# anonymous-author-918/deq-mpc-corl

Hardware: AMD Instinct MI355X
Metric: QP solves/sec at (B,T=20,nx=13,nu=4) (higher is better)
Workload: dtype f32

## Files before the change

### deq-mpc-corl_amd/csrc/alqp_quad.hip

```cpp
#include <hip/hip_runtime.h>

#include "alqp_quad.hpp"
#include "alqp_dims.hpp"
#include "alqp_launch.hpp"

#if defined(ALQP_QUAD_F32) == defined(ALQP_QUAD_F64)
#error "compile alqp_quad.hip with exactly one of -DALQP_QUAD_F32, -DALQP_QUAD_F64"
#endif

namespace alqp {

#ifndef ALQP_FUSE_LS
#define ALQP_FUSE_LS 1
#endif
#ifdef ALQP_PHASE_TIMING
__device__ unsigned long long g_phase_cycles[10];
#define QSTAMP(b) qd.stamp(b)
#else
#define QSTAMP(b)
#endif
template <typename real, int NX, int NU, bool TRACE, class Dyn = NoDyn>
__global__ __launch_bounds__(64) __attribute__((amdgpu_waves_per_eu(1, 1))) void k_solve_lin_quad(SolveArgs<real> a, TraceArgs<real> tr, real *ws) {
    using C = QCfg<real, NX, NU>;
    constexpr bool NL = Dyn::ID != 0;
#ifndef ALQP_FUSE_LS_F64
#define ALQP_FUSE_LS_F64 1
#endif
    constexpr bool FUSE_LS = ALQP_FUSE_LS && (sizeof(real) == 4 || ALQP_FUSE_LS_F64) && !NL;
    constexpr int N = C::N;
    if (a.skip && *a.skip != 0.0) return;
    const int lane = threadIdx.x, qi = lane >> 2;
    const int b_raw = blockIdx.x * 16 + qi;
    const bool active = b_raw < a.B;
    {
        int stag = a.stagger;
        const int mode = (a.flags >> 20) & 0xf;
        if ((a.flags >> 24) & 0xff) stag = (a.flags >> 24) & 0xff;
        if (stag > 0) {
            const unsigned hw = __builtin_amdgcn_s_getreg(4 | (0 << 6) | (31 << 11));
            int simd = (hw >> 4) & 3;
            if (mode == 1) simd = simd * 16 + ((hw >> 8) & 0xf);
            if (mode == 2) simd &= 1;
            if (mode == 3) simd = blockIdx.x & 1;
            if (mode == 4) simd = (simd & 1) ^ (blockIdx.x & 1);
            if (mode == 5) simd = (hw >> 8) & 3;
            for (int i = 0; i < simd * stag; ++i) __builtin_amdgcn_s_sleep(16);
        }
    }
#ifdef ALQP_ALIAS_ALL
    const int b = (active ? b_raw : a.B - 1) % ALQP_ALIAS_ALL;
#else
    const int b = active ? b_raw : a.B - 1;
#endif
    const int T = a.T, M = C::M(T);

    Quad<real, NX, NU> qd;
    __shared__ real w_lds[QCfg<real, NX, NU>::WLDS_WORDS];
    qd.wl = w_lds + threadIdx.x;
    qd.q = lane & 3;
    qd.T = T;
    qd.active = active;
    qd.gQd = a.Qd + (size_t)b * T * N;
    qd.gq = a.q + (size_t)b * T * N;
    qd.gF = a.F + (size_t)b * (T - 1) * NX * N;
    qd.gc = a.c + (size_t)b * (T - 1) * NX;
    qd.gx0 = a.x0 + (size_t)b * NX;
    qd.gulo = a.ulo + (size_t)b * a.sb_u;
    qd.guhi = a.uhi + (size_t)b * a.sb_u;
    qd.st_u = a.st_u;
    qd.gz = a.z + (size_t)b * T * N;
    qd.glam = a.lam + (size_t)b * M;
    qd.rec = ws + C::rec_base(b, T);
    qd.gFw = const_cast<real *>(qd.gF);
    qd.dyn_h = a.dyn_h;
    qd.rho = a.rho[b];
    qd.info = 0;
    real phi_prev = a.phi[b];
#ifdef ALQP_PHASE_TIMING
    for (int i = 0; i < 10; ++i) qd.tacc[i] = 0;
#endif
    QSTAMP(-1);
    if (!(a.flags & ALQP_WS_PRIMED)) {
        if constexpr (NL) qd.stage_in(false, false);
        else qd.stage_in(a.max_newton == 0 || a.al_iter == 0 || (a.flags & ALQP_EXIT_IN_KERNEL) ||
                         (!C::PHI0_FWD && (a.flags & ALQP_INIT_MERIT)));
    }
    const bool ref_exit = (a.flags & ALQP_EXIT_IN_KERNEL) != 0;
    int gphase = 0;

    int step_id = 0;
    bool pend = false;
// ... 84 lines not shown
        if (ref_exit && a.newton_counts && blockIdx.x == 0 && lane == 0) a.newton_counts[it] = grid_barrier_timed_out(a.exit_scratch) ? -1 : n_done;
        bad = 0;
        qd.template iter_end<Dyn>(alpha_pend, pend, (a.flags & ALQP_DUAL_UPDATE) != 0, (real)a.rho_scale, it + 1 == a.al_iter,
                    phi_next, rn2, bad);
        pend = false;
    }
    if (a.al_iter <= 0) {
        rn2 = qd.rplus2(bad);
        qd.stage_out();
    }
#ifdef ALQP_PHASE_TIMING
    QSTAMP(9);
    if (lane == 0)
        for (int i = 0; i < 10; ++i) atomicAdd(&g_phase_cycles[i], qd.tacc[i]);
#endif
    if (active && qd.q == 0) {
        a.rho[b] = qd.rho;
        a.phi[b] = phi_prev;
        if (a.rnorm2) a.rnorm2[b] = rn2;
        if (a.info && qd.info && a.info[b] == 0) a.info[b] = qd.info;
        if (a.status) a.status[b] = bad ? 0 : 1;
    }
}

template <typename real, int NX, int NU>
__global__ __launch_bounds__(64) __attribute__((amdgpu_waves_per_eu(1, 1))) void k_backward_quad(BwdArgs<real> a, real *ws) {
    using C = QCfg<real, NX, NU>;
    constexpr int N = C::N;
    const int lane = threadIdx.x, qi = lane >> 2;
    const int b_raw = blockIdx.x * 16 + qi;
    const bool active = b_raw < a.B;
    const int b = active ? b_raw : a.B - 1;
    const int T = a.T;
    Quad<real, NX, NU> qd;
    __shared__ real w_lds[QCfg<real, NX, NU>::WLDS_WORDS];
    qd.wl = w_lds + threadIdx.x;
    qd.q = lane & 3;
    qd.T = T;
    qd.active = active;
    qd.gF = a.F + (size_t)b * (T - 1) * NX * N;
    qd.gQd = nullptr; qd.gq = nullptr; qd.gc = nullptr; qd.gx0 = nullptr; qd.gulo = nullptr; qd.guhi = nullptr;
    qd.st_u = 0;
    qd.gz = nullptr; qd.glam = nullptr;
    qd.rec = ws + C::rec_base(b, T);
    qd.rho = a.rho[b];
    qd.info = 0;
    qd.solve_forward(a.gbar + (size_t)b * T * N);
    real unused[20];
    qd.template backward<false>(unused);
    if (active) {
        const real *zf = a.z_final + (size_t)b * T * N;
        real *qg = a.q_grad + (size_t)b * T * N;
        real *Qg = a.Qd_grad + (size_t)b * T * N;
        for (int t = 0; t < T; ++t)
            for (int j = qd.q; j < N; j += 4) {
                const real w = qd.recp(t)[C::wn(C::oY, j)];
                qg[t * N + j] = w;
                Qg[t * N + j] = w * zf[t * N + j];
            }
    }
}

template <typename real, int NX, int NU>
__global__ __launch_bounds__(64) __attribute__((amdgpu_waves_per_eu(1, 1))) void k_newton_step_quad(StepArgs<real> a, real *ws) {
    using C = QCfg<real, NX, NU>;
    constexpr int N = C::N, SW = C::SW;
    const int lane = threadIdx.x, qi = lane >> 2;
    const int b_raw = blockIdx.x * 16 + qi;
    const bool active = b_raw < a.B;
    const int b = active ? b_raw : a.B - 1;
    const int T = a.T, M = C::M(T) + T * a.nobs;
    Quad<real, NX, NU> qd;
    __shared__ real w_lds[QCfg<real, NX, NU>::WLDS_WORDS];
    qd.wl = w_lds + threadIdx.x;
    qd.q = lane & 3;
    qd.T = T;
    qd.active = active;
    qd.gQd = a.Qd + (size_t)b * T * N;
    qd.gq = a.q + (size_t)b * T * N;
    qd.gF = a.F + (size_t)b * (T - 1) * NX * N;
    qd.gc = nullptr;
    qd.gx0 = a.x0 + (size_t)b * NX;
    qd.gulo = a.ulo + (size_t)b * a.sb_u;
    qd.guhi = a.uhi + (size_t)b * a.sb_u;
    qd.st_u = a.st_u;
    qd.gz = const_cast<real *>(a.z) + (size_t)b * T * N;
    qd.glam = const_cast<real *>(a.lam) + (size_t)b * M;
    qd.rec = ws + C::rec_base(b, T);
    qd.gFw = const_cast<real *>(qd.gF);
    qd.dyn_h = 0;
    qd.rho = a.rho[b];
    qd.info = 0;
    qd.nobs = a.nobs;
    qd.gobs = a.nobs > 0 ? a.obs + (size_t)b * T * a.nobs * 3 : nullptr;
    qd.obs_r2 = a.obs_r2;
    qd.no_init = a.no_init != 0;
    const real *gxn = a.xnext + (size_t)b * (T - 1) * NX;
    real *tg = (a.g_out && active) ? a.g_out + (size_t)b * T * N : nullptr;
    qd.template forward<true>(tg, real(0), false, nullptr, gxn);
    real unused[20];
    qd.template backward<false>(unused, a.d_out + (size_t)b * T * N);
    if (active) {
        if (qd.q == 0 && a.info && qd.info && a.info[b] == 0) a.info[b] = qd.info;
    }
}


// ... 69 lines not shown
```

### deq-mpc-corl_amd/csrc/alqp_quad.hpp

```cpp
#pragma once
#include <hip/hip_runtime.h>

#include <type_traits>

#include "alqp_team.hpp"
#include "alqp_dyn.hpp"

namespace alqp {

template <int Q>
__device__ inline float qb(float v) {
    return __builtin_bit_cast(float, __builtin_amdgcn_mov_dpp(__builtin_bit_cast(int, v), Q * 0x55, 0xF, 0xF, true));
}
template <int Q>
__device__ inline double qb(double v) {
    long long b = __builtin_bit_cast(long long, v);
    int lo = __builtin_amdgcn_mov_dpp((int)(b & 0xffffffffll), Q * 0x55, 0xF, 0xF, true);
    int hi = __builtin_amdgcn_mov_dpp((int)(b >> 32), Q * 0x55, 0xF, 0xF, true);
    return __builtin_bit_cast(double, ((long long)hi << 32) | (unsigned int)lo);
}
template <typename real>
__device__ inline real qbv(real v, int src) {
    switch (src & 3) {
        case 0: return qb<0>(v);
        case 1: return qb<1>(v);
        case 2: return qb<2>(v);
        default: return qb<3>(v);
    }
}
template <int CTRL>
__device__ inline float qperm(float v) {
    return __builtin_bit_cast(float, __builtin_amdgcn_mov_dpp(__builtin_bit_cast(int, v), CTRL, 0xF, 0xF, true));
}
template <int CTRL>
__device__ inline double qperm(double v) {
    long long b = __builtin_bit_cast(long long, v);
    int lo = __builtin_amdgcn_mov_dpp((int)(b & 0xffffffffll), CTRL, 0xF, 0xF, true);
    int hi = __builtin_amdgcn_mov_dpp((int)(b >> 32), CTRL, 0xF, 0xF, true);
    return __builtin_bit_cast(double, ((long long)hi << 32) | (unsigned int)lo);
}
template <typename real>
__device__ inline real qsum(real v) {
    v += qperm<0xB1>(v);
    v += qperm<0x4E>(v);
    return v;
}
__device__ inline int qor(int v) {
    v |= __builtin_amdgcn_mov_dpp(v, 0xB1, 0xF, 0xF, true);
    v |= __builtin_amdgcn_mov_dpp(v, 0x4E, 0xF, 0xF, true);
    return v;
}
template <typename real>
__device__ inline real sel4(real a0, real a1, real a2, real a3, int q) {
    real lo = (q & 1) ? a1 : a0, hi = (q & 1) ? a3 : a2;
    return (q & 2) ? hi : lo;
}

struct __attribute__((packed, aligned(4))) f4u { float x, y, z, w; };
struct __attribute__((packed, aligned(8))) d4u { double x, y, z, w; };
__device__ inline void gld4(const float *p, float &a, float &b, float &c, float &d) {
    f4u t = *reinterpret_cast<const f4u *>(p);
// ... 1 lines not shown
}
__device__ inline void gld4(const double *p, double &a, double &b, double &c, double &d) {
    d4u t = *reinterpret_cast<const d4u *>(p);
    a = t.x; b = t.y; c = t.z; d = t.w;
}
__device__ inline void gst4(float *p, float a, float b, float c, float d) {
    f4u t; t.x = a; t.y = b; t.z = c; t.w = d;
    *reinterpret_cast<f4u *>(p) = t;
}
__device__ inline void gst4(double *p, double a, double b, double c, double d) {
    d4u t; t.x = a; t.y = b; t.z = c; t.w = d;
    *reinterpret_cast<d4u *>(p) = t;
}
template <int LEN, typename real>
__device__ inline void gload(const real *p, real (&dst)[LEN]) {
#pragma unroll
    for (int c = 0; c + 4 <= LEN; c += 4) gld4(p + c, dst[c], dst[c + 1], dst[c + 2], dst[c + 3]);
#pragma unroll
    for (int c = (LEN / 4) * 4; c < LEN; ++c) dst[c] = p[c];
}

#ifndef ALQP_W_LDS
#define ALQP_W_LDS 1
#endif
#ifndef ALQP_EXP_NOQ
#define ALQP_EXP_NOQ 0
#endif
#ifndef ALQP_EXP_NORS
#define ALQP_EXP_NORS 0
#endif
#ifndef ALQP_EXP_NOL
#define ALQP_EXP_NOL 0
#endif
template <typename real, int SW, int N, bool IN_LDS>
struct WPanel {
    real a[SW][N];
    __device__ __forceinline__ real (&operator[](int s))[N] { return a[s]; }
    __device__ __forceinline__ const real (&operator[](int s) const)[N] { return a[s]; }
};
template <typename real, int N>
struct WRowLds {
    real *p;
    __device__ __forceinline__ real &operator[](int k) const { return p[k * 64]; }
};
template <typename real, int SW, int N>
struct WPanel<real, SW, N, true> {
    real *base;
    __device__ __forceinline__ WRowLds<real, N> operator[](int s) const { return WRowLds<real, N>{base + s * N * 64}; }
};
template <int LEN, typename real>
__device__ __forceinline__ void gload(const real *p, WRowLds<real, LEN> row) {
    real tmp[LEN];
    gload<LEN>(p, tmp);
#pragma unroll
    for (int k = 0; k < LEN; ++k) row[k] = tmp[k];
}

struct NoDyn {
    static constexpr int ID = 0;
};

struct Fld {
    int h, t;
};
template <int H, int T>
struct FldT {
// ... 15 lines not shown
    static constexpr int NX = NX_, NU = NU_, N = NX_ + NU_;
    static constexpr int SH = (N + 3) / 4;
    static constexpr int SW = (NX + 3) / 4;
    static constexpr int SY = SH;
    static constexpr int HT = 2 * SH * (SH + 1);
    __host__ __device__ static constexpr int hidx(int s, int j) { return 2 * s * (s + 1) + j; }
    static constexpr int ST = 2 * SW * (SW + 1);
    static constexpr int BLK = 64 / (int)sizeof(real);
#ifndef ALQP_REC_IL_F32
#define ALQP_REC_IL_F32 2
#endif
    static constexpr int IL = sizeof(real) == 4 ? ALQP_REC_IL_F32 : 1;
    static_assert(IL == 1 || BLK == 16, "groups of 16 words are 64-byte blocks");
    __host__ __device__ static constexpr int w(int x) { return (x / 16) * (16 * IL) + x % 16; }
    static constexpr int NLAST = N - 4 * (SH - 1);
    __host__ __device__ static constexpr int lanes_of(int s) { return s == SH - 1 ? NLAST : 4; }
    __host__ __device__ static constexpr int lstride(int s) { return lanes_of(s) == 3 ? 16 : 4 * lanes_of(s); }
    __host__ __device__ static constexpr int lbase(int s) {
        int o = 0;
        for (int i = 0; i < s; ++i) o += (i + 1) * lstride(i);
        return o;
    }
    static constexpr int LW = lbase(SH);
    static constexpr bool PHI0_FWD = sizeof(real) == 4;
#ifndef ALQP_S_AFTER_F32
#define ALQP_S_AFTER_F32 0
#endif
    static constexpr bool S_AFTER = sizeof(real) == 8 || ALQP_S_AFTER_F32;
#ifndef ALQP_W_LDS_F32
#define ALQP_W_LDS_F32 0
#endif
    static constexpr bool W_LDS = ALQP_W_LDS && (sizeof(real) == 8 || ALQP_W_LDS_F32);
    static constexpr int WLDS_WORDS = W_LDS ? SW * N * 64 : 1;
    __host__ __device__ static constexpr int p4(int x) { return (x + 3) & ~3; }
    static constexpr int NF = 9;
    __host__ __device__ static constexpr int fslots(int i) { return (i <= 1 || i == 6 || i == 7) ? SY : (i == 5 ? 4 : SW); }
    static constexpr int oL = 2 * 16 * (SY / 4);
    __host__ __device__ static constexpr int tail_at(int i) {
        int g = (oL + LW + 15) & ~15, o = 0;
        for (int k = 0; k < NF; ++k) {
            const int r = fslots(k) % 4;
            if (r > 0 && o + r > 4) { g += 16; o = 0; }
            if (k == i) return g + o;
            o += r;
        }
        return o > 0 ? g + 16 : g;
    }
    __host__ __device__ static constexpr int head_at(int i) {
        if (i < 2) return i * 16 * (SY / 4);
        int o = tail_at(NF);
        for (int k = 2; k < i; ++k) o += 16 * (fslots(k) / 4);
        return o;
    }
    static constexpr FldT<head_at(0), tail_at(0)> oY{};
    static constexpr FldT<head_at(1), tail_at(1)> oZ{};
    static constexpr FldT<head_at(2), tail_at(2)> oR{};
    static constexpr FldT<head_at(3), tail_at(3)> oS{};
    static constexpr FldT<head_at(4), tail_at(4)> oLE{};
    static_assert(NU <= 4, "the u-slot layout holds one control per lane");
    static constexpr FldT<head_at(5), tail_at(5)> oUS{};
    static constexpr FldT<head_at(6), tail_at(6)> oQ{};
    static constexpr FldT<head_at(7), tail_at(7)> oq{};
    static constexpr FldT<head_at(8), tail_at(8)> oC{};
    static constexpr int RECW = (head_at(NF) + 31) & ~31;
    static_assert(IL == 1 || RECW % 16 == 0, "whole groups per record");
    template <int S>
    __host__ __device__ static constexpr int lp(int m, int q) {
        return m < 4 * (S / 4) ? 16 * (m / 4) + 4 * q + m % 4 : 16 * (S / 4) + q * (S % 4) + m - 4 * (S / 4);
    }
    template <int S>
    __host__ __device__ static constexpr int fw(Fld f, int p) {
        return p < 16 * (S / 4) ? w(f.h + p) : w(f.t + 4 * ((p - 16 * (S / 4)) / (S % 4)) + (p - 16 * (S / 4)) % (S % 4));
    }
    __host__ __device__ static constexpr int pn(int k) { return lp<SY>(k >> 2, k & 3); }
    __host__ __device__ static constexpr int px(int r) { return lp<SW>(r >> 2, r & 3); }
    __host__ __device__ static constexpr int wn(Fld f, int k) { return fw<SY>(f, pn(k)); }
    __host__ __device__ static constexpr int M(int T) { return T * NX + 2 * T * NU; }
    static constexpr int RSTR = RECW * IL;
    __host__ __device__ static constexpr size_t rec_base(int b, int T) { return (size_t)(b / IL) * T * RSTR + (size_t)(b % IL) * 16; }
    __host__ __device__ static constexpr size_t ws_words(int B, int T) { return (size_t)((B + IL - 1) / IL) * T * RSTR; }
    __host__ static bool ws_covers(int B, int T) {
        return rec_base(B - 1, T) + (size_t)(T - 1) * RSTR + w(RECW - 1) + 1 <= ws_words(B, T);
    }
};

template <typename real, int NX, int NU>
struct Quad {
    using C = QCfg<real, NX, NU>;
    static constexpr int N = C::N, SH = C::SH, SW = C::SW, SY = C::SY, HT = C::HT, ST = C::ST, RECW = C::RECW;

    int q, T;
    bool active;
    const real *gQd, *gq, *gF, *gc, *gx0, *gulo, *guhi;
    long st_u;
    real *gz, *glam, *rec;
    real rho;
    int info;
    real *wl;
    using WT = WPanel<real, SW, N, C::W_LDS>;
    __device__ __forceinline__ WT wpanel() const {
        if constexpr (C::W_LDS) return WT{wl};
        else return WT{};
    }
    real *gFw;
    real dyn_h;
    const real *gobs;
    int nobs;
    real obs_r2;
    bool no_init;

    __device__ __forceinline__ real uhi(int t, int j) const { return guhi[t * st_u + j]; }
    __device__ __forceinline__ real ulo(int t, int j) const { return gulo[t * st_u + j]; }
    __device__ __forceinline__ real *recp(int t) const { return rec + (size_t)t * C::RSTR; }
#ifdef ALQP_PHASE_TIMING
    unsigned long long tacc[10], tlast;
    __device__ __forceinline__ void stamp(int bucket) {
        unsigned long long now;
        __builtin_amdgcn_sched_barrier(0);
        asm volatile("s_waitcnt vmcnt(0)\n\ts_memtime %0\n\ts_waitcnt lgkmcnt(0)" : "=s"(now)::"memory");
        __builtin_amdgcn_sched_barrier(0);
        if (bucket >= 0) tacc[bucket] += now - tlast;
        tlast = now;
// ... 88 lines not shown
        for (int m = 0; m < SL; ++m) {
            const int k = 4 * m + q;
            const real x = src[(4 * m + 3 < LEN || k < LEN) ? k : LEN - 1];
            v[m] = (4 * m + 3 < LEN || k < LEN) ? x : real(0);
        }
    }
    template <int LEN, int SL>
    __device__ __forceinline__ void st_own_ext(real *dst, const real (&v)[SL]) const {
#pragma unroll
        for (int m = 0; m < SL; ++m)
            if (4 * m + 3 < LEN || 4 * m + q < LEN) dst[4 * m + q] = v[m];
    }

    __device__ __forceinline__ int own_ju() const { return (q - NX) & 3; }
    __device__ __forceinline__ void ld_own_us(const real *rp, real &lu, real &ll, real &bu, real &bl) const {
        gld4(rp + C::w(C::oUS.h) + 4 * q, lu, ll, bu, bl);
    }
    __device__ __forceinline__ void st_own_us(real *rp, real lu, real ll, real bu, real bl) const {
        gst4(rp + C::w(C::oUS.h) + 4 * q, lu, ll, bu, bl);
    }
    __device__ __forceinline__ void ld_rep_us(const real *rp, real (&lu)[NU], real (&ll)[NU], real (&bu)[NU], real (&bl)[NU]) const {
        real w[16];
        ld_field<4>(rp + C::oUS, w);
#pragma unroll
        for (int ju = 0; ju < NU; ++ju) {
            const int ql = (NX + ju) & 3;
            lu[ju] = w[4 * ql];
            ll[ju] = w[4 * ql + 1];
            bu[ju] = w[4 * ql + 2];
            bl[ju] = w[4 * ql + 3];
        }
    }

    __device__ __forceinline__ void load_F_rows(int t, WT &W) const {
        const real *Fg = gF + (size_t)t * NX * N;
#pragma unroll
        for (int s = 0; s < SW; ++s) {
            const int r = 4 * s + q;
            const int rc = (4 * s + 3 < NX) ? r : (r < NX ? r : NX - 1);
            gload<N>(Fg + rc * N, W[s]);
            if (4 * s + 3 >= NX) {
                const real m = r < NX ? real(1) : real(0);
#pragma unroll
                for (int k = 0; k < N; ++k) W[s][k] *= m;
            }
        }
    }
    template <int LEN>
    __device__ __forceinline__ void copy_slice(const real *src, real *dst) const {
#pragma unroll
        for (int c = 0; 16 * c < LEN; ++c) {
            const int w0 = 16 * c + 4 * q;
            if (16 * c + 15 < LEN || w0 + 3 < LEN) {
                real a, b, cc, d;
                gld4(src + w0, a, b, cc, d);
                gst4(dst + w0, a, b, cc, d);
            } else {
#pragma unroll
                for (int w = 0; w < 4; ++w)
                    if (w0 + w < LEN) dst[w0 + w] = src[w0 + w];
            }
        }
    }
    __device__ __forceinline__ void stage_in(bool with_residual, bool have_c = true) {
#pragma unroll 2
        for (int t = 0; t < T; ++t) {
            const bool dyn = t < T - 1;
            real *rp = recp(t);
            if (active) {
                real vn[SY], vx[SW];
                ld_own_ext<N>(gz + t * N, vn);
                st_own_n(rp + C::oZ, vn);
                ld_own_ext<N>(gQd + t * N, vn);
                st_own_n(rp + C::oQ, vn);
                ld_own_ext<N>(gq + t * N, vn);
                st_own_n(rp + C::oq, vn);
                ld_own_ext<NX>(glam + t * NX, vx);
                st_own_x(rp + C::oLE, vx);
                {
                    const int ju = own_ju(), jc = ju < NU ? ju : 0;
                    const real *lb = glam + T * NX + t * 2 * NU;
                    const real a0 = lb[jc], a1 = lb[NU + jc], a2 = guhi[t * st_u + jc], a3 = gulo[t * st_u + jc];
                    const bool has = ju < NU;
                    st_own_us(rp, has ? a0 : real(0), has ? a1 : real(0), has ? a2 : real(0), has ? a3 : real(0));
                }
                if (dyn && have_c) ld_own_ext<NX>(gc + t * NX, vx);
                else {
#pragma unroll
                    for (int s = 0; s < SW; ++s) vx[s] = 0;
                }
                if (have_c) st_own_x(rp + C::oC, vx);
            }
            if (with_residual) {
                WT W = wpanel();
                real zt[N];
                load_F_rows(dyn ? t : (T > 1 ? T - 2 : 0), W);
                gload<N>(gz + t * N, zt);
                real rr[SW];
#pragma unroll
                for (int s = 0; s < SW; ++s) {
                    const int r = 4 * s + q;
                    rr[s] = 0;
                    if (4 * s + 3 < NX || r < NX) {
                        real xn = dyn ? gc[t * NX + r] : real(0);
#pragma unroll
                        for (int k = 0; k < N; ++k) xn = fma_(W[s][k], zt[k], xn);
                        rr[s] = dyn ? gz[(t + 1) * N + r] - xn : gz[r] - gx0[r];
                    }
                }
                if (active) st_own_x(rp + C::oR, rr);
            }
        }
    }
    __device__ __forceinline__ void stage_out() {
        if (!active) return;
#pragma unroll 2
        for (int t = 0; t < T; ++t) {
            const real *rp = recp(t);
            real vn[SY], vx[SW];
            ld_own_n(rp + C::oZ, vn);
            st_own_ext<N>(gz + t * N, vn);
            ld_own_x(rp + C::oLE, vx);
            st_own_ext<NX>(glam + t * NX, vx);
            {
                real lu, ll, bu, bl;
                ld_own_us(rp, lu, ll, bu, bl);
                const int ju = own_ju();
                if (ju < NU) {
                    glam[T * NX + t * 2 * NU + ju] = lu;
                    glam[T * NX + t * 2 * NU + NU + ju] = ll;
// ... 145 lines not shown
#pragma unroll
        for (int s = 0; s < SW; ++s) Sy[s] = 0;
        {
            real z0[SW], xi[SW], li[SW], r0[SW];
            if constexpr (EXT) {
                ld_own_ext<NX>(gz, z0);
                ld_own_ext<NX>(glam + (T - 1) * NX, li);
            } else {
                ld_ownx_of_n(recp(0) + C::oZ, z0);
                ld_own_x(recp(T - 1) + C::oLE, li);
            }
            ld_own_ext<NX>(gx0, xi);
            if (pending) {
                real d0[SW];
                ld_ownx_of_n(recp(0) + C::oY, d0);
#pragma unroll
                for (int s = 0; s < SW; ++s) z0[s] = fma_(alpha, d0[s], z0[s]);
            }
#pragma unroll
            for (int s = 0; s < SW; ++s) {
                bool valid = 4 * s + 3 < NX || 4 * s + q < NX;
                if constexpr (EXT) valid = valid && !no_init;
                const real r = valid ? z0[s] - xi[s] : real(0);
                vpo[s] = valid ? fma_(rho, r, li[s]) : real(0);
                if constexpr (C::PHI0_FWD) mdist += valid ? fma_(fma_(real(0.5) * rho, r, li[s]), r, real(0)) : real(0);
                Syo[s] = 0;
                r0[s] = r;
            }
            if (!EXT && active) st_own_x(recp(T - 1) + C::oR, r0);
        }
        for (int t = 0; t < T; ++t) {
            const bool dyn = t < T - 1;
            WT W = wpanel();
            real Y[N];
            real dio[SY];
            real v[SW];
            real zs[SY];
            real hob[3] = {0, 0, 0};
            real *rp = recp(t);
            {
                real zt[N];
                real Qo[SY], qo[SY];
                real cs[SW], zn[SW], lm[SW];
                real lu, ll, bu, bl;
                const int td = dyn ? t : (T > 1 ? T - 2 : 0);
                const real *rn = recp(td + 1);
                if constexpr (EXT) {
                    ld_own_ext<N>(gz + t * N, zs);
                    ld_own_ext<N>(gQd + t * N, Qo);
                    ld_own_ext<N>(gq + t * N, qo);
                    load_F_rows(td, W);
                    ld_own_ext<NX>(gxn + td * NX, cs);
                    ld_own_ext<NX>(gz + (td + 1) * N, zn);
                    ld_own_ext<NX>(glam + td * NX, lm);
                    const int ju = own_ju(), jc = ju < NU ? ju : 0;
                    const real *lb = glam + T * NX + t * (2 * NU + nobs);
                    const bool has = ju < NU;
                    lu = has ? lb[jc] : real(0);
                    ll = has ? lb[NU + jc] : real(0);
                    bu = has ? guhi[t * st_u + jc] : real(0);
                    bl = has ? gulo[t * st_u + jc] : real(0);
                } else {
                    ld_own_n(rp + C::oZ, zs);
                    if constexpr (ALQP_EXP_NOQ) { for (int m = 0; m < SY; ++m) Qo[m] = real(1); }
                    else ld_own_n(rp + C::oQ, Qo);
                    ld_own_n(rp + C::oq, qo);
                    load_F_rows(td, W);
                    ld_own_x(rp + C::oC, cs);
                    ld_ownx_of_n(rn + C::oZ, zn);
                    ld_own_x(rp + C::oLE, lm);
                    ld_own_us(rp, lu, ll, bu, bl);
                }
                if (pending) {
                    real dt[SY], dn[SW];
                    ld_own_n(rp + C::oY, dt);
                    ld_ownx_of_n(rn + C::oY, dn);
#pragma unroll
                    for (int m = 0; m < SY; ++m) zs[m] = fma_(alpha, dt[m], zs[m]);
#pragma unroll
                    for (int s = 0; s < SW; ++s) zn[s] = fma_(alpha, dn[s], zn[s]);
                }
                ALQP_STAMP(0);
#pragma unroll
                for (int k = 0; k < N; ++k) zt[k] = qbv(zs[k >> 2], k);
                real rro[SW];
                if (!dyn) {
#pragma unroll
                    for (int s = 0; s < SW; ++s)
#pragma unroll
                        for (int k = 0; k < N; ++k) W[s][k] = 0;
                }
#pragma unroll
                for (int s = 0; s < SW; ++s) {
                    const int r = 4 * s + q;
                    real xn = cs[s];
                    if constexpr (!EXT) {
#pragma unroll
                        for (int k = 0; k < N; ++k) xn = fma_(W[s][k], zt[k], xn);
                    }
                    const real rr = zn[s] - xn;
                    const bool ok = dyn && r < NX;
                    v[s] = ok ? fma_(rho, rr, lm[s]) : real(0);
                    rro[s] = ok ? rr : real(0);
                    if constexpr (C::PHI0_FWD) mdist += ok ? fma_(fma_(real(0.5) * rho, rr, lm[s]), rr, real(0)) : real(0);
                }
                if (!ALQP_EXP_NORS && !EXT && dyn && active) st_own_x(rp + C::oR, rro);
                constexpr int MU0 = NX / 4;
                real zu = 0;
#pragma unroll
                for (int m = MU0; m < SY; ++m) zu = (4 * m + q >= NX && 4 * m + q < N) ? zs[m] : zu;
                const real vu = zu - bu, vl = bl - zu;
                const real au = vu >= 0 ? real(1) : real(0), al = vl >= 0 ? real(1) : real(0);
                const real cu = fmax_(vu, real(0)), cl = fmax_(vl, real(0));
                const real gu = fma_(rho, cu, lu) - fma_(rho, cl, ll);
                const real du = rho * (au + al);
                if constexpr (C::PHI0_FWD)
                    mdist += own_ju() < NU ? fma_(lu, vu, ll * vl) + real(0.5) * rho * fma_(cu, cu, cl * cl) : real(0);
                real go[SY];
#pragma unroll
                for (int m = 0; m < SY; ++m) {
                    const int j = 4 * m + q;
                    const bool isx = (4 * m + 3 < NX) ? true : (4 * m >= NX ? false : j < NX);
                    const bool isu = (4 * m + 3 < NX) ? false : (j >= NX && j < N);
                    real g = fma_(Qo[m], zs[m], qo[m]);
// ... 12 lines not shown
                if constexpr (EXT && NX >= 3) {
                    if (nobs > 0) {
                        const real *lk = glam + T * NX + t * (2 * NU + nobs) + 2 * NU;
                        real gob = 0;
                        for (int k = 0; k < nobs; ++k) {
                            const real *o = gobs + (size_t)(t * nobs + k) * 3;
                            const real d0 = zt[0] - o[0], d1 = zt[1] - o[1], d2 = zt[2] - o[2];
                            const real ck = obs_r2 - fma_(d0, d0, fma_(d1, d1, d2 * d2));
                            const real dh = q == 0 ? d0 : (q == 1 ? d1 : d2);
                            gob = fma_(fma_(rho, ck > 0 ? ck : real(0), lk[k]), real(-2) * dh, gob);
                            if (ck >= 0) {
                                const real w4 = real(4) * rho * dh;
                                hob[0] = fma_(w4, d0, hob[0]); hob[1] = fma_(w4, d1, hob[1]); hob[2] = fma_(w4, d2, hob[2]);
                            }
                        }
                        go[0] += q < 3 ? gob : real(0);
                    }
                }
#pragma unroll
                for (int m = 0; m < SY; ++m) {
                    const bool isx = (4 * m + 3 < NX) ? true : (4 * m >= NX ? false : 4 * m + q < NX);
                    go[m] = -go[m] - (isx ? Syo[m < SW ? m : 0] : real(0));
                }
                real fv[N];
#pragma unroll
                for (int j = 0; j < N; ++j) {
                    real p = 0;
                    if (dyn) {
#pragma unroll
                        for (int s = 0; s < SW; ++s) p = fma_(W[s][j], v[s], p);
                        p = qsum(p);
                    }
                    fv[j] = p;
                    Y[j] = qbv(go[j >> 2], j) + p;
                }
                if (g_out) {
                    real fo[SY];
                    own_of<N, SY>(fv, fo);
#pragma unroll
                    for (int m = 0; m < SY; ++m) {
                        const bool isx = (4 * m + 3 < NX) ? true : (4 * m >= NX ? false : 4 * m + q < NX);
                        if (4 * m + 3 < N || 4 * m + q < N)
                            g_out[t * N + 4 * m + q] = -(go[m] + fo[m]) - (isx ? Syo[m < SW ? m : 0] : real(0));
                    }
                }
            }
            real H[HT];
#pragma unroll
            for (int i = 0; i < HT; ++i) H[i] = 0;
#pragma unroll
            for (int s = 0; s < SH; ++s)
#pragma unroll
                for (int c = 0; c < 4; ++c)
                    if (4 * s + c < N) H[C::hidx(s, 4 * s + c)] = (q == c) ? dio[s] : real(0);
            if constexpr (EXT && NX >= 3) {
                if (nobs > 0 && q < 3) {
#pragma unroll
                    for (int j = 0; j < 3; ++j) H[C::hidx(0, j)] += hob[j];
                }
            }
            if (t > 0) {
#pragma unroll
                for (int s = 0; s < SW; ++s)
#pragma unroll
                    for (int b = 0; b < 4 * s + 4; ++b)
                        if (b < NX) H[C::hidx(s, b)] -= S[C::hidx(s, b)];
            }
#pragma unroll
            for (int i = 0; i < ST; ++i) S[i] = 0;
#pragma unroll
            for (int s = 0; s < SW; ++s) Sy[s] = 0;
#pragma unroll
            for (int s = 0; s < SW; ++s)
#pragma unroll
                for (int k = 0; k < N; ++k) W[s][k] *= -rho;
            if (dyn) {
                const real irho = real(1) / rho;
#pragma unroll
                for (int r = 0; r < NX; ++r) {
                    real fr[N];
#pragma unroll
                    for (int j = 0; j < N; ++j) fr[j] = qbv(W[r >> 2][j], r);
#pragma unroll
                    for (int s = 0; s < SH; ++s) {
                        real fi = sel4(fr[4 * s], (4 * s + 1 < N) ? fr[(4 * s + 1 < N) ? 4 * s + 1 : 0] : real(0),
                                       (4 * s + 2 < N) ? fr[(4 * s + 2 < N) ? 4 * s + 2 : 0] : real(0),
                                       (4 * s + 3 < N) ? fr[(4 * s + 3 < N) ? 4 * s + 3 : 0] : real(0), q) * irho;
#pragma unroll
                        for (int j = 0; j < 4 * s + 4; ++j)
                            if (j < N) H[C::hidx(s, j)] = fma_(fi, fr[j], H[C::hidx(s, j)]);
                    }
                }
            }
            ALQP_STAMP(1);
            real ipv[C::S_AFTER ? N : 1];
#pragma unroll
            for (int j = 0; j < N; ++j) {
                const real p = qbv(H[C::hidx(j >> 2, j)], j);
                if (!(p > 0) && info == 0) info = t * N + j + 1;
                const real ip = rcp_(fabs_(p));
                if constexpr (C::W_LDS) {
                    constexpr int KB = 8;
                    real wj[SW];
#pragma unroll
                    for (int s = 0; s < SW; ++s) wj[s] = W[s][j];
#pragma unroll
                    for (int k0 = j + 1; k0 < N; k0 += KB) {
                        real wv[KB][SW];
#pragma unroll
                        for (int kk = 0; kk < KB; ++kk)
#pragma unroll
                            for (int s = 0; s < SW; ++s)
                                if (k0 + kk < N) wv[kk][s] = W[s][k0 + kk];
                        __builtin_amdgcn_sched_barrier(0);
#pragma unroll
                        for (int kk = 0; kk < KB; ++kk) {
                            const int k = k0 + kk;
                            if (k < N) {
                                const real lkj = qbv(H[C::hidx(k >> 2, j)], k) * ip;
#pragma unroll
                                for (int s = (k >> 2); s < SH; ++s) H[C::hidx(s, k)] = fma_(-H[C::hidx(s, j)], lkj, H[C::hidx(s, k)]);
#pragma unroll
                                for (int s = 0; s < SW; ++s) W[s][k] = fma_(-wj[s], lkj, wv[kk][s]);
                                Y[k] = fma_(-Y[j], lkj, Y[k]);
                            }
                        }
                    }
                } else {
#pragma unroll
                for (int k = j + 1; k < N; ++k) {
                    const real lkj = qbv(H[C::hidx(k >> 2, j)], k) * ip;
#pragma unroll
                    for (int s = (k >> 2); s < SH; ++s) H[C::hidx(s, k)] = fma_(-H[C::hidx(s, j)], lkj, H[C::hidx(s, k)]);
#pragma unroll
                    for (int s = 0; s < SW; ++s) W[s][k] = fma_(-W[s][j], lkj, W[s][k]);
                    Y[k] = fma_(-Y[j], lkj, Y[k]);
                }
                }
                if constexpr (C::S_AFTER) ipv[j] = ip;
                if (!C::S_AFTER && dyn) {
#pragma unroll
                    for (int b = 0; b < NX; ++b) {
                        const real wbj = qbv(W[b >> 2][j], b) * ip;
#pragma unroll
                        for (int s = (b >> 2); s < SW; ++s) S[C::hidx(s, b)] = fma_(W[s][j], wbj, S[C::hidx(s, b)]);
                    }
                    const real yip = Y[j] * ip;
#pragma unroll
                    for (int s = 0; s < SW; ++s) Sy[s] = fma_(W[s][j], yip, Sy[s]);
                }
                H[C::hidx(j >> 2, j)] = (q == (j & 3)) ? ip : H[C::hidx(j >> 2, j)];
            }
            ALQP_STAMP(2);
            if (active) {
                if (!(ALQP_EXP_NOL && t >= T - ALQP_EXP_NOL))
#pragma unroll
                for (int s = 0; s < SH; ++s)
#pragma unroll
                    for (int c = 0; c <= s; ++c)
                        if (C::lanes_of(s) == 4 || q < C::lanes_of(s))
                            gst4(lchunk(rp, s, c, q), H[C::hidx(s, 4 * c)],
                                 H[C::hidx(s, 4 * c + 1)], H[C::hidx(s, 4 * c + 2)], H[C::hidx(s, 4 * c + 3)]);
                real yo[SY];
                own_of<N, SY>(Y, yo);
                st_own_n(rp + C::oY, yo);
                if (pending) st_own_n(rp + C::oZ, zs);
            }

            if constexpr (C::S_AFTER) {
                if (dyn) {
#pragma unroll
                    for (int j = 0; j < N; ++j) {
#pragma unroll
                        for (int b = 0; b < NX; ++b) {
                            const real wbj = qbv(W[b >> 2][j], b) * ipv[j];
#pragma unroll
                            for (int s = (b >> 2); s < SW; ++s) S[C::hidx(s, b)] = fma_(W[s][j], wbj, S[C::hidx(s, b)]);
                        }
                        const real yip = Y[j] * ipv[j];
#pragma unroll
                        for (int s = 0; s < SW; ++s) Sy[s] = fma_(W[s][j], yip, Sy[s]);
                    }
                }
            }
#pragma unroll
            for (int s = 0; s < SW; ++s) {
                vpo[s] = v[s];
                Syo[s] = Sy[s];
            }
            ALQP_STAMP(3);
        }
        if constexpr (C::PHI0_FWD) { if (phi0) *phi0 = qsum(mdist); }
    }

    template <bool LS>
    __device__ __forceinline__ void backward(real (&phi)[20], real *d_ext = nullptr) {
        constexpr int MU0 = NX / 4;
        real c0 = 0, c1 = 0, c2 = 0;
        real acc[20];
        real rvT[SW], lvT[SW];
#pragma unroll
        for (int k = 0; k < 20; ++k) acc[k] = 0;
#pragma unroll
        for (int s = 0; s < SW; ++s) rvT[s] = lvT[s] = 0;
        real dxn[NX];
#pragma unroll
        for (int j = 0; j < NX; ++j) dxn[j] = 0;
        for (int t = T - 1; t >= 0; --t) {
            const bool dyn = t < T - 1;
            real *rp = recp(t);
            real H[HT];
            if (ALQP_EXP_NOL && t >= T - ALQP_EXP_NOL) {
#pragma unroll
                for (int i = 0; i < HT; ++i) H[i] = real(1);
            } else
#pragma unroll
            for (int s = 0; s < SH; ++s)
#pragma unroll
                for (int c = 0; c <= s; ++c) {
                    const int ql = (C::lanes_of(s) == 4 || q < C::lanes_of(s)) ? q : 0;
                    gld4(lchunk(rp, s, c, ql), H[C::hidx(s, 4 * c)],
                         H[C::hidx(s, 4 * c + 1)], H[C::hidx(s, 4 * c + 2)], H[C::hidx(s, 4 * c + 3)]);
                }
            real yo[SY];
            ld_own_n(rp + C::oY, yo);
            real Y[N];
#pragma unroll
            for (int j = 0; j < N; ++j) Y[j] = qbv(yo[j >> 2], j);
            WT W = wpanel();
            load_F_rows(dyn ? t : (T > 1 ? T - 2 : 0), W);
            real zz[SY], QQ[SY], qq[SY], rv[SW], lv[SW];
            real lu = 0, ll = 0, bu = 0, bl = 0;
            if constexpr (LS) {
                ld_own_n(rp + C::oZ, zz);
                if constexpr (ALQP_EXP_NOQ) { for (int m = 0; m < SY; ++m) QQ[m] = real(1); }
                else ld_own_n(rp + C::oQ, QQ);
                ld_own_n(rp + C::oq, qq);
                ld_own_us(rp, lu, ll, bu, bl);
                if constexpr (ALQP_EXP_NORS) { for (int s = 0; s < SW; ++s) rv[s] = real(0); }
                else ld_own_x(rp + C::oR, rv);
                ld_own_x(rp + C::oLE, lv);
            }
            ALQP_STAMP(4);
            real dxs[SW];
#pragma unroll
            for (int s = 0; s < SW; ++s)
                dxs[s] = sel4(dxn[4 * s], (4 * s + 1 < NX) ? dxn[(4 * s + 1 < NX) ? 4 * s + 1 : 0] : real(0),
                              (4 * s + 2 < NX) ? dxn[(4 * s + 2 < NX) ? 4 * s + 2 : 0] : real(0),
                              (4 * s + 3 < NX) ? dxn[(4 * s + 3 < NX) ? 4 * s + 3 : 0] : real(0), q);
            if (dyn) {
                real vv[N];
#pragma unroll
                for (int j = 0; j < N; ++j) {
                    real p = 0;
#pragma unroll
                    for (int s = 0; s < SW; ++s) p = fma_(W[s][j], dxs[s], p);
                    vv[j] = qsum(p);
                }
#pragma unroll
                for (int j = 0; j < N; ++j) {
                    const real wj = vv[j] * qbv(H[C::hidx(j >> 2, j)], j);
#pragma unroll
                    for (int k = j + 1; k < N; ++k) vv[k] = fma_(-qbv(H[C::hidx(k >> 2, j)], k), wj, vv[k]);
                }
#pragma unroll
                for (int j = 0; j < N; ++j) Y[j] = fma_(rho, vv[j], Y[j]);
            }
#pragma unroll
            for (int i = N - 1; i >= 0; --i) {
                const real di = Y[i] * qbv(H[C::hidx(i >> 2, i)], i);
                Y[i] = di;
#pragma unroll
                for (int j = 0; j < i; ++j) Y[j] = fma_(-qbv(H[C::hidx(i >> 2, j)], i), di, Y[j]);
            }
            if (active) {
                real down[SY];
// ... 86 lines not shown
                c1 = fma_(fma_(rho, rr, lm), ss, c1);
                c2 = fma_(real(0.5) * rho * ss, ss, c2);
            }
            c0 = qsum(c0);
            c1 = qsum(c1);
            c2 = qsum(c2);
            real alpha = 1;
#pragma unroll
            for (int k = 0; k < 20; ++k) {
                phi[k] = qsum(acc[k]) + fma_(alpha, fma_(alpha, c2, c1), c0);
                alpha *= real(0.5);
            }
        }
    }

    __device__ __forceinline__ void solve_forward(const real *gbar) {
        real e[N];
#pragma unroll
        for (int j = 0; j < N; ++j) e[j] = 0;
        for (int t = 0; t < T; ++t) {
            real *rp = recp(t);
            real H[HT];
#pragma unroll
            for (int s = 0; s < SH; ++s)
#pragma unroll
                for (int c = 0; c <= s; ++c) {
                    const int ql = (C::lanes_of(s) == 4 || q < C::lanes_of(s)) ? q : 0;
                    gld4(lchunk(rp, s, c, ql), H[C::hidx(s, 4 * c)],
                         H[C::hidx(s, 4 * c + 1)], H[C::hidx(s, 4 * c + 2)], H[C::hidx(s, 4 * c + 3)]);
                }
            real Y[N];
            gload<N>(gbar + t * N, Y);
            WT W = wpanel();
            load_F_rows(t > 0 ? t - 1 : 0, W);
#pragma unroll
            for (int j = 0; j < N; ++j) Y[j] = -Y[j];
            if (t > 0) {
                real cpl[SW];
#pragma unroll
                for (int s = 0; s < SW; ++s) {
                    real p = 0;
#pragma unroll
                    for (int k = 0; k < N; ++k) p = fma_(W[s][k], e[k], p);
                    cpl[s] = p;
                }
#pragma unroll
                for (int j = 0; j < NX; ++j) Y[j] = fma_(rho, qbv(cpl[j >> 2], j), Y[j]);
            }
#pragma unroll
            for (int j = 0; j < N; ++j) {
                const real yj = Y[j] * qbv(H[C::hidx(j >> 2, j)], j);
#pragma unroll
                for (int k = j + 1; k < N; ++k) Y[k] = fma_(-qbv(H[C::hidx(k >> 2, j)], k), yj, Y[k]);
            }
            if (active) {
                real yo[SY];
                own_of<N, SY>(Y, yo);
                st_own_n(rp + C::oY, yo);
            }
#pragma unroll
            for (int j = 0; j < N; ++j) e[j] = Y[j];
#pragma unroll
            for (int i = N - 1; i >= 0; --i) {
                const real ei = e[i] * qbv(H[C::hidx(i >> 2, i)], i);
                e[i] = ei;
#pragma unroll
                for (int j = 0; j < i; ++j) e[j] = fma_(-qbv(H[C::hidx(i >> 2, j)], i), ei, e[j]);
// ... 230 lines not shown
```

Baseline: 5.965 million.

## Stage F dynamics rows through LDS with coalesced 16-byte chunk loads

```diff
diff --git a/deq-mpc-corl_amd/csrc/alqp_quad.hip b/deq-mpc-corl_amd/csrc/alqp_quad.hip
--- a/deq-mpc-corl_amd/csrc/alqp_quad.hip
+++ b/deq-mpc-corl_amd/csrc/alqp_quad.hip
@@ -54,9 +54,10 @@
 #endif
     const int T = a.T, M = C::M(T);
 
-    Quad<real, NX, NU> qd;
-    __shared__ real w_lds[QCfg<real, NX, NU>::WLDS_WORDS];
-    qd.wl = w_lds + threadIdx.x;
+    constexpr bool FST = C::F_STAGE && !NL;
+    Quad<real, NX, NU, FST> qd;
+    __shared__ alignas(FST ? 16 : alignof(real)) real w_lds[FST ? C::FLDS_WORDS : C::WLDS_WORDS];
+    qd.wl = FST ? w_lds + qi * C::FM::S : w_lds + threadIdx.x;
     qd.q = lane & 3;
     qd.T = T;
     qd.active = active;
@@ -207,9 +208,10 @@
     const bool active = b_raw < a.B;
     const int b = active ? b_raw : a.B - 1;
     const int T = a.T;
-    Quad<real, NX, NU> qd;
-    __shared__ real w_lds[QCfg<real, NX, NU>::WLDS_WORDS];
-    qd.wl = w_lds + threadIdx.x;
+    constexpr bool FST = C::F_STAGE;
+    Quad<real, NX, NU, FST> qd;
+    __shared__ alignas(FST ? 16 : alignof(real)) real w_lds[FST ? C::FLDS_WORDS : C::WLDS_WORDS];
+    qd.wl = FST ? w_lds + qi * C::FM::S : w_lds + threadIdx.x;
     qd.q = lane & 3;
     qd.T = T;
     qd.active = active;
@@ -245,9 +247,10 @@
     const bool active = b_raw < a.B;
     const int b = active ? b_raw : a.B - 1;
     const int T = a.T, M = C::M(T) + T * a.nobs;
-    Quad<real, NX, NU> qd;
-    __shared__ real w_lds[QCfg<real, NX, NU>::WLDS_WORDS];
-    qd.wl = w_lds + threadIdx.x;
+    constexpr bool FST = C::F_STAGE;
+    Quad<real, NX, NU, FST> qd;
+    __shared__ alignas(FST ? 16 : alignof(real)) real w_lds[FST ? C::FLDS_WORDS : C::WLDS_WORDS];
+    qd.wl = FST ? w_lds + qi * C::FM::S : w_lds + threadIdx.x;
     qd.q = lane & 3;
     qd.T = T;
     qd.active = active;
diff --git a/deq-mpc-corl_amd/csrc/alqp_quad.hpp b/deq-mpc-corl_amd/csrc/alqp_quad.hpp
--- a/deq-mpc-corl_amd/csrc/alqp_quad.hpp
+++ b/deq-mpc-corl_amd/csrc/alqp_quad.hpp
@@ -94,6 +94,53 @@
 #ifndef ALQP_EXP_NOL
 #define ALQP_EXP_NOL 0
 #endif
+#ifndef ALQP_EXP_FCHUNK
+#define ALQP_EXP_FCHUNK 0
+#endif
+
+#ifndef ALQP_F_STAGE
+#define ALQP_F_STAGE 1
+#endif
+template <int NX, int N>
+struct FStageMap {
+    static constexpr int WORDS = NX * N, SW = (NX + 3) / 4;
+    static constexpr int NCH_MIN = (WORDS + 3) / 4;
+    static constexpr int NCH_MAX = (WORDS + 6) / 4;
+    static constexpr int CPL = (NCH_MAX + 3) / 4;
+    __host__ __device__ static constexpr int nch(int o) { return (o + WORDS + 3) >> 2; }
+    __host__ __device__ static constexpr int chunk(int c, int q, int o) {
+        const int ch = 4 * c + q, last = nch(o) - 1;
+        return ch < last ? ch : last;
+    }
+    __host__ __device__ static constexpr int row(int s, int q) { return 4 * s + q < NX ? 4 * s + q : NX - 1; }
+    __host__ __device__ static constexpr int rd(int o, int s, int q, int k) { return o + N * row(s, q) + k; }
+    __host__ __device__ static constexpr int worst_banks(int S) {
+        int worst = 0;
+        for (int h = 0; h < 2; ++h)
+            for (int s = 0; s < SW; ++s) {
+                int tot[32] = {};
+                for (int i = 8 * h; i < 8 * h + 8; ++i) {
+                    int mx[32] = {};
+                    for (int o = 0; o < 4; ++o) {
+                        int cnt[32] = {};
+                        for (int q = 0; q < 4; ++q)
+                            if (q == 0 || row(s, q) != row(s, q - 1)) ++cnt[(i * S + rd(o, s, q, 0)) & 31];
+                        for (int b = 0; b < 32; ++b) mx[b] = cnt[b] > mx[b] ? cnt[b] : mx[b];
+                    }
+                    for (int b = 0; b < 32; ++b) tot[b] += mx[b];
+                }
+                for (int b = 0; b < 32; ++b) worst = tot[b] > worst ? tot[b] : worst;
+            }
+        return worst;
+    }
+    __host__ __device__ static constexpr int pick_S() {
+        int S = (WORDS + 6 + 3) / 4 * 4;
+        while (worst_banks(S) > 4) S += 4;
+        return S;
+    }
+    static constexpr int S = pick_S();
+    static_assert(S >= 4 * NCH_MAX && S % 4 == 0, "the image holds every chunk, 16-byte aligned");
+};
 template <typename real, int SW, int N, bool IN_LDS>
 struct WPanel {
     real a[SW][N];
@@ -175,6 +222,12 @@
 #endif
     static constexpr bool W_LDS = ALQP_W_LDS && (sizeof(real) == 8 || ALQP_W_LDS_F32);
     static constexpr int WLDS_WORDS = W_LDS ? SW * N * 64 : 1;
+    using FM = FStageMap<NX_, NX_ + NU_>;
+    __host__ __device__ static constexpr bool f_stage_pays() {
+        return !((NX_ == 8 && NU_ == 2) || (NX_ == 12 && NU_ == 4) || (NX_ == 14 && NU_ == 4));
+    }
+    static constexpr bool F_STAGE = ALQP_F_STAGE && !W_LDS && sizeof(real) == 4 && f_stage_pays();
+    static constexpr int FLDS_WORDS = 16 * FM::S;
     __host__ __device__ static constexpr int p4(int x) { return (x + 3) & ~3; }
     static constexpr int NF = 9;
     __host__ __device__ static constexpr int fslots(int i) { return (i <= 1 || i == 6 || i == 7) ? SY : (i == 5 ? 4 : SW); }
@@ -227,10 +280,12 @@
     }
 };
 
-template <typename real, int NX, int NU>
+template <typename real, int NX, int NU, bool FST = false>
 struct Quad {
     using C = QCfg<real, NX, NU>;
+    using FM = typename C::FM;
     static constexpr int N = C::N, SH = C::SH, SW = C::SW, SY = C::SY, HT = C::HT, ST = C::ST, RECW = C::RECW;
+    static_assert(!FST || (C::F_STAGE && !C::W_LDS), "the staging image takes the place of the W panel in LDS");
 
     int q, T;
     bool active;
@@ -385,8 +440,25 @@
         }
     }
 
-    __device__ __forceinline__ void load_F_rows(int t, WT &W) const {
+    struct FChunks {
+        real v[FST ? 4 * FM::CPL : 1];
+        int o;
+    };
+    struct __attribute__((aligned(16))) r4a { real x, y, z, w; };
+    __device__ __forceinline__ void load_F_rows(int t, WT &W, FChunks &fc) const {
         const real *Fg = gF + (size_t)t * NX * N;
+        if constexpr (FST) {
+            const unsigned long long A = (unsigned long long)Fg;
+            fc.o = (int)(A >> 2) & 3;
+            const real *Fa = (const real *)(A & ~15ull) + 4 * q;
+#pragma unroll
+            for (int c = 0; c < FM::CPL; ++c) {
+                const real *p = (4 * c + 3 < FM::NCH_MIN) ? Fa + 16 * c : Fa - 4 * q + 4 * FM::chunk(c, q, fc.o);
+                const r4a t4 = *reinterpret_cast<const r4a *>(p);
+                fc.v[4 * c] = t4.x; fc.v[4 * c + 1] = t4.y; fc.v[4 * c + 2] = t4.z; fc.v[4 * c + 3] = t4.w;
+            }
+            return;
+        }
 #pragma unroll
         for (int s = 0; s < SW; ++s) {
             const int r = 4 * s + q;
@@ -397,6 +469,42 @@
 #pragma unroll
                 for (int k = 0; k < N; ++k) W[s][k] *= m;
             }
+        }
+    }
+    __device__ __forceinline__ void finish_F_rows(const FChunks &fc, WT &W) const {
+        if constexpr (FST) {
+            __builtin_amdgcn_sched_barrier(0);
+#if ALQP_EXP_FCHUNK
+#pragma unroll
+            for (int s = 0; s < SW; ++s)
+#pragma unroll
+                for (int k = 0; k < N; ++k) W[s][k] = fc.v[(s * N + k) % (4 * FM::CPL)];
+#else
+            real *img = wl;
+            wave_sync();
+#pragma unroll
+            for (int c = 0; c < FM::CPL; ++c) {
+                const int ch = (4 * c + 3 < FM::NCH_MIN) ? 4 * c + q : FM::chunk(c, q, fc.o);
+                r4a t4;
+                t4.x = fc.v[4 * c]; t4.y = fc.v[4 * c + 1]; t4.z = fc.v[4 * c + 2]; t4.w = fc.v[4 * c + 3];
+                *reinterpret_cast<r4a *>(img + 4 * ch) = t4;
+            }
+            wave_sync();
+            const real *rb = img + fc.o + N * q;
+#pragma unroll
+            for (int s = 0; s < SW; ++s) {
+                const int r = 4 * s + q;
+                const real *rs = (4 * s + 3 < NX) ? rb + 4 * s * N : img + FM::rd(fc.o, s, q, 0);
+#pragma unroll
+                for (int k = 0; k < N; ++k) W[s][k] = rs[k];
+                if (4 * s + 3 >= NX) {
+                    const real m = r < NX ? real(1) : real(0);
+#pragma unroll
+                    for (int k = 0; k < N; ++k) W[s][k] *= m;
+                }
+            }
+            wave_sync();
+#endif
         }
     }
     template <int LEN>
@@ -447,8 +555,10 @@
             if (with_residual) {
                 WT W = wpanel();
                 real zt[N];
-                load_F_rows(dyn ? t : (T > 1 ? T - 2 : 0), W);
+                FChunks fc;
+                load_F_rows(dyn ? t : (T > 1 ? T - 2 : 0), W, fc);
                 gload<N>(gz + t * N, zt);
+                finish_F_rows(fc, W);
                 real rr[SW];
 #pragma unroll
                 for (int s = 0; s < SW; ++s) {
@@ -671,13 +781,14 @@
                 real Qo[SY], qo[SY];
                 real cs[SW], zn[SW], lm[SW];
                 real lu, ll, bu, bl;
+                FChunks fc;
                 const int td = dyn ? t : (T > 1 ? T - 2 : 0);
                 const real *rn = recp(td + 1);
                 if constexpr (EXT) {
                     ld_own_ext<N>(gz + t * N, zs);
                     ld_own_ext<N>(gQd + t * N, Qo);
                     ld_own_ext<N>(gq + t * N, qo);
-                    load_F_rows(td, W);
+                    load_F_rows(td, W, fc);
                     ld_own_ext<NX>(gxn + td * NX, cs);
                     ld_own_ext<NX>(gz + (td + 1) * N, zn);
                     ld_own_ext<NX>(glam + td * NX, lm);
@@ -693,7 +804,7 @@
                     if constexpr (ALQP_EXP_NOQ) { for (int m = 0; m < SY; ++m) Qo[m] = real(1); }
                     else ld_own_n(rp + C::oQ, Qo);
                     ld_own_n(rp + C::oq, qo);
-                    load_F_rows(td, W);
+                    load_F_rows(td, W, fc);
                     ld_own_x(rp + C::oC, cs);
                     ld_ownx_of_n(rn + C::oZ, zn);
                     ld_own_x(rp + C::oLE, lm);
@@ -709,6 +820,7 @@
                     for (int s = 0; s < SW; ++s) zn[s] = fma_(alpha, dn[s], zn[s]);
                 }
                 ALQP_STAMP(0);
+                finish_F_rows(fc, W);
 #pragma unroll
                 for (int k = 0; k < N; ++k) zt[k] = qbv(zs[k >> 2], k);
                 real rro[SW];
@@ -992,7 +1104,8 @@
 #pragma unroll
             for (int j = 0; j < N; ++j) Y[j] = qbv(yo[j >> 2], j);
             WT W = wpanel();
-            load_F_rows(dyn ? t : (T > 1 ? T - 2 : 0), W);
+            FChunks fc;
+            load_F_rows(dyn ? t : (T > 1 ? T - 2 : 0), W, fc);
             real zz[SY], QQ[SY], qq[SY], rv[SW], lv[SW];
             real lu = 0, ll = 0, bu = 0, bl = 0;
             if constexpr (LS) {
@@ -1006,6 +1119,7 @@
                 ld_own_x(rp + C::oLE, lv);
             }
             ALQP_STAMP(4);
+            finish_F_rows(fc, W);
             real dxs[SW];
 #pragma unroll
             for (int s = 0; s < SW; ++s)
@@ -1158,7 +1272,9 @@
             real Y[N];
             gload<N>(gbar + t * N, Y);
             WT W = wpanel();
-            load_F_rows(t > 0 ? t - 1 : 0, W);
+            FChunks fc;
+            load_F_rows(t > 0 ? t - 1 : 0, W, fc);
+            finish_F_rows(fc, W);
 #pragma unroll
             for (int j = 0; j < N; ++j) Y[j] = -Y[j];
             if (t > 0) {
```

Result: no change. 5.973 million, median of 2 (+0.1%).

## Keep forward RHS in owned layout and fuse H initialization with Schur subtraction

Applied to the files above, without the earlier changes.

```diff
diff --git a/deq-mpc-corl_amd/csrc/alqp_quad.hpp b/deq-mpc-corl_amd/csrc/alqp_quad.hpp
--- a/deq-mpc-corl_amd/csrc/alqp_quad.hpp
+++ b/deq-mpc-corl_amd/csrc/alqp_quad.hpp
@@ -27,6 +27,13 @@
         case 2: return qb<2>(v);
         default: return qb<3>(v);
     }
+}
+#ifndef ALQP_EXP_SCALE_FIRST
+#define ALQP_EXP_SCALE_FIRST 0
+#endif
+template <typename real>
+__device__ inline real qbv_scaled(real v, real ip, int src) {
+    return ALQP_EXP_SCALE_FIRST ? qbv(v * ip, src) : qbv(v, src) * ip;
 }
 template <int CTRL>
 __device__ inline float qperm(float v) {
@@ -231,6 +238,7 @@
 struct Quad {
     using C = QCfg<real, NX, NU>;
     static constexpr int N = C::N, SH = C::SH, SW = C::SW, SY = C::SY, HT = C::HT, ST = C::ST, RECW = C::RECW;
+    __host__ __device__ static constexpr bool h_ff_only(int s, int j) { return j < 4 * s && !(s < SW && j < NX); }
 
     int q, T;
     bool active;
@@ -660,7 +668,7 @@
         for (int t = 0; t < T; ++t) {
             const bool dyn = t < T - 1;
             WT W = wpanel();
-            real Y[N];
+            real yo[SY];
             real dio[SY];
             real v[SW];
             real zs[SY];
@@ -712,12 +720,6 @@
 #pragma unroll
                 for (int k = 0; k < N; ++k) zt[k] = qbv(zs[k >> 2], k);
                 real rro[SW];
-                if (!dyn) {
-#pragma unroll
-                    for (int s = 0; s < SW; ++s)
-#pragma unroll
-                        for (int k = 0; k < N; ++k) W[s][k] = 0;
-                }
 #pragma unroll
                 for (int s = 0; s < SW; ++s) {
                     const int r = 4 * s + q;
@@ -796,11 +798,12 @@
                         p = qsum(p);
                     }
                     fv[j] = p;
-                    Y[j] = qbv(go[j >> 2], j) + p;
-                }
+                }
+                real fo[SY];
+                own_of<N, SY>(fv, fo);
+#pragma unroll
+                for (int m = 0; m < SY; ++m) yo[m] = go[m] + fo[m];
                 if (g_out) {
-                    real fo[SY];
-                    own_of<N, SY>(fv, fo);
 #pragma unroll
                     for (int m = 0; m < SY; ++m) {
                         const bool isx = (4 * m + 3 < NX) ? true : (4 * m >= NX ? false : 4 * m + q < NX);
@@ -811,33 +814,26 @@
             }
             real H[HT];
 #pragma unroll
-            for (int i = 0; i < HT; ++i) H[i] = 0;
-#pragma unroll
             for (int s = 0; s < SH; ++s)
 #pragma unroll
-                for (int c = 0; c < 4; ++c)
-                    if (4 * s + c < N) H[C::hidx(s, 4 * s + c)] = (q == c) ? dio[s] : real(0);
-            if constexpr (EXT && NX >= 3) {
-                if (nobs > 0 && q < 3) {
-#pragma unroll
-                    for (int j = 0; j < 3; ++j) H[C::hidx(0, j)] += hob[j];
-                }
-            }
-            if (t > 0) {
-#pragma unroll
-                for (int s = 0; s < SW; ++s)
-#pragma unroll
-                    for (int b = 0; b < 4 * s + 4; ++b)
-                        if (b < NX) H[C::hidx(s, b)] -= S[C::hidx(s, b)];
-            }
+                for (int j = 0; j < 4 * s + 4; ++j) {
+                    if (j >= N) { H[C::hidx(s, j)] = 0; continue; }
+                    if (h_ff_only(s, j)) continue;
+                    real dg = (j >= 4 * s) ? ((q == j - 4 * s) ? dio[s] : real(0)) : real(0);
+                    if constexpr (EXT && NX >= 3) {
+                        if (s == 0 && j < 3) dg = (nobs > 0 && q < 3) ? dg + hob[j < 3 ? j : 0] : dg;
+                    }
+                    H[C::hidx(s, j)] = (s < SW && j < NX) ? dg - S[C::hidx(s < SW ? s : 0, j)] : dg;
+                }
 #pragma unroll
             for (int i = 0; i < ST; ++i) S[i] = 0;
 #pragma unroll
             for (int s = 0; s < SW; ++s) Sy[s] = 0;
+            const real wsc_t = dyn ? -rho : real(0);
 #pragma unroll
             for (int s = 0; s < SW; ++s)
 #pragma unroll
-                for (int k = 0; k < N; ++k) W[s][k] *= -rho;
+                for (int k = 0; k < N; ++k) W[s][k] *= wsc_t;
             if (dyn) {
                 const real irho = real(1) / rho;
 #pragma unroll
@@ -852,9 +848,15 @@
                                        (4 * s + 3 < N) ? fr[(4 * s + 3 < N) ? 4 * s + 3 : 0] : real(0), q) * irho;
 #pragma unroll
                         for (int j = 0; j < 4 * s + 4; ++j)
-                            if (j < N) H[C::hidx(s, j)] = fma_(fi, fr[j], H[C::hidx(s, j)]);
-                    }
-                }
+                            if (j < N) H[C::hidx(s, j)] = (r == 0 && h_ff_only(s, j)) ? fi * fr[j] : fma_(fi, fr[j], H[C::hidx(s, j)]);
+                    }
+                }
+            } else {
+#pragma unroll
+                for (int s = 0; s < SH; ++s)
+#pragma unroll
+                    for (int j = 0; j < 4 * s; ++j)
+                        if (j < N && h_ff_only(s, j)) H[C::hidx(s, j)] = 0;
             }
             ALQP_STAMP(1);
             real ipv[C::S_AFTER ? N : 1];
@@ -881,35 +883,39 @@
                         for (int kk = 0; kk < KB; ++kk) {
                             const int k = k0 + kk;
                             if (k < N) {
-                                const real lkj = qbv(H[C::hidx(k >> 2, j)], k) * ip;
+                                const real lkj = qbv_scaled(H[C::hidx(k >> 2, j)], ip, k);
 #pragma unroll
                                 for (int s = (k >> 2); s < SH; ++s) H[C::hidx(s, k)] = fma_(-H[C::hidx(s, j)], lkj, H[C::hidx(s, k)]);
 #pragma unroll
                                 for (int s = 0; s < SW; ++s) W[s][k] = fma_(-wj[s], lkj, wv[kk][s]);
-                                Y[k] = fma_(-Y[j], lkj, Y[k]);
                             }
                         }
                     }
                 } else {
 #pragma unroll
                 for (int k = j + 1; k < N; ++k) {
-                    const real lkj = qbv(H[C::hidx(k >> 2, j)], k) * ip;
+                    const real lkj = qbv_scaled(H[C::hidx(k >> 2, j)], ip, k);
 #pragma unroll
                     for (int s = (k >> 2); s < SH; ++s) H[C::hidx(s, k)] = fma_(-H[C::hidx(s, j)], lkj, H[C::hidx(s, k)]);
 #pragma unroll
                     for (int s = 0; s < SW; ++s) W[s][k] = fma_(-W[s][j], lkj, W[s][k]);
-                    Y[k] = fma_(-Y[j], lkj, Y[k]);
-                }
+                }
+                }
+                const real yip = qbv(yo[j >> 2] * ip, j);
+#pragma unroll
+                for (int m = (j >> 2); m < SY; ++m) {
+                    const real yn = fma_(-H[C::hidx(m, j)], yip, yo[m]);
+                    if (m > (j >> 2)) yo[m] = yn;
+                    else if ((j & 3) < 3) yo[m] = (q > (j & 3)) ? yn : yo[m];
                 }
                 if constexpr (C::S_AFTER) ipv[j] = ip;
                 if (!C::S_AFTER && dyn) {
 #pragma unroll
                     for (int b = 0; b < NX; ++b) {
-                        const real wbj = qbv(W[b >> 2][j], b) * ip;
+                        const real wbj = qbv_scaled(W[b >> 2][j], ip, b);
 #pragma unroll
                         for (int s = (b >> 2); s < SW; ++s) S[C::hidx(s, b)] = fma_(W[s][j], wbj, S[C::hidx(s, b)]);
                     }
-                    const real yip = Y[j] * ip;
 #pragma unroll
                     for (int s = 0; s < SW; ++s) Sy[s] = fma_(W[s][j], yip, Sy[s]);
                 }
@@ -925,8 +931,7 @@
                         if (C::lanes_of(s) == 4 || q < C::lanes_of(s))
                             gst4(lchunk(rp, s, c, q), H[C::hidx(s, 4 * c)],
                                  H[C::hidx(s, 4 * c + 1)], H[C::hidx(s, 4 * c + 2)], H[C::hidx(s, 4 * c + 3)]);
-                real yo[SY];
-                own_of<N, SY>(Y, yo);
+                if constexpr (N % 4 != 0) yo[SY - 1] = (4 * (SY - 1) + q < N) ? yo[SY - 1] : real(0);
                 st_own_n(rp + C::oY, yo);
                 if (pending) st_own_n(rp + C::oZ, zs);
             }
@@ -935,15 +940,18 @@
                 if (dyn) {
 #pragma unroll
                     for (int j = 0; j < N; ++j) {
+                        real wj[SW];
+#pragma unroll
+                        for (int s = 0; s < SW; ++s) wj[s] = W[s][j];
 #pragma unroll
                         for (int b = 0; b < NX; ++b) {
-                            const real wbj = qbv(W[b >> 2][j], b) * ipv[j];
-#pragma unroll
-                            for (int s = (b >> 2); s < SW; ++s) S[C::hidx(s, b)] = fma_(W[s][j], wbj, S[C::hidx(s, b)]);
+                            const real wbj = qbv_scaled(wj[b >> 2], ipv[j], b);
+#pragma unroll
+                            for (int s = (b >> 2); s < SW; ++s) S[C::hidx(s, b)] = fma_(wj[s], wbj, S[C::hidx(s, b)]);
                         }
-                        const real yip = Y[j] * ipv[j];
-#pragma unroll
-                        for (int s = 0; s < SW; ++s) Sy[s] = fma_(W[s][j], yip, Sy[s]);
+                        const real yip = qbv(yo[j >> 2] * ipv[j], j);
+#pragma unroll
+                        for (int s = 0; s < SW; ++s) Sy[s] = fma_(wj[s], yip, Sy[s]);
                     }
                 }
             }
```

New measurement: 6.007 million before, 5.925 million after. -1.4%, worse.
